# wangys16/FreeSplat

Measured on AMD Instinct MI355X. Metric: rendered views/sec @ 968x1296, 1.0M Gaussians, higher is better.
Workload: dtype f32

## Files before the change

freesplat_amd/csrc/raster_fwd.hip:

```cpp
#include <stdlib.h>

#include <type_traits>

#include "fs_common.h"
#include "raster_host.h"

namespace fs {

template <int M>
__device__ __forceinline__ uint32_t lane_xor(uint32_t v)
{
    if constexpr (M == 1) return (uint32_t)__builtin_amdgcn_mov_dpp((int)v, 0xB1, 0xF, 0xF, true);
    else if constexpr (M == 2) return (uint32_t)__builtin_amdgcn_mov_dpp((int)v, 0x4E, 0xF, 0xF, true);
    else if constexpr (M == 3) return (uint32_t)__builtin_amdgcn_mov_dpp((int)v, 0x1B, 0xF, 0xF, true);
    else if constexpr (M < 32) return (uint32_t)__builtin_amdgcn_ds_swizzle((int)v, (M << 10) | 0x1F);
    else return (uint32_t)__shfl_xor((int)v, M, 64);
}
template <int M>
__device__ __forceinline__ unsigned long long lane_xor64(unsigned long long v)
{
    const uint32_t lo = lane_xor<M>((uint32_t)v), hi = lane_xor<M>((uint32_t)(v >> 32));
    return ((unsigned long long)hi << 32) | lo;
}

// ... 200 lines not shown
        const float fx = (float)d.W / (2.0f * tanfovx), fy = (float)d.H / (2.0f * tanfovy);
        float c3[6];
#pragma unroll
        for (int k = 0; k < 6; ++k) c3[k] = c_in[k];
        if (rescale) {
            const float s2 = wscale * wscale;
#pragma unroll
            for (int k = 0; k < 6; ++k) c3[k] = c3[k] * s2;
        }
        const Cov2D cv = project_cov(view, p, c3, fx, fy, tanfovx, tanfovy);
        const float det = cv.a * cv.c - cv.b * cv.b;
        if (det != 0.0f) {
            const float det_inv = 1.0f / det;
            const float cA = cv.c * det_inv, cB = -cv.b * det_inv, cC = cv.a * det_inv;
            const float mid = 0.5f * (cv.a + cv.c);
            const float sq = sqrtf(fmaxf(0.1f, mid * mid - det));
            const float l1 = mid + sq, l2 = mid - sq;
            const float my_radius = ceilf(3.0f * sqrtf(fmaxf(l1, l2)));
            const float px = ((ndcx + 1.0f) * (float)d.W - 1.0f) * 0.5f;
            const float py = ((ndcy + 1.0f) * (float)d.H - 1.0f) * 0.5f;
            const int r = (int)my_radius;
            const int gx = (d.W + kTile - 1) / kTile, gy = (d.H + kTile - 1) / kTile;
            const int x0 = min(gx, max(0, (int)((px - (float)r) / (float)kTile)));
            const int y0 = min(gy, max(0, (int)((py - (float)r) / (float)kTile)));
            const int x1 = min(gx, max(0, (int)((px + (float)r + (float)(kTile - 1)) / (float)kTile)));
            const int y1 = min(gy, max(0, (int)((py + (float)r + (float)(kTile - 1)) / (float)kTile)));
            if ((x1 - x0) * (y1 - y0) > 0) {
                float rgb[3];
                if (colors) {
                    rgb[0] = colors[3 * i];
                    rgb[1] = colors[3 * i + 1];
                    rgb[2] = colors[3 * i + 2];
                } else {
                    float3 dir = make_float3(p.x - campos[0], p.y - campos[1], p.z - campos[2]);
                    const float len = sqrtf(dir.x * dir.x + dir.y * dir.y + dir.z * dir.z);
                    dir.x = dir.x / len; dir.y = dir.y / len; dir.z = dir.z / len;
                    switch (d.sh_degree) {
                        case 0: eval_sh<0>(sh, dir, rgb, o.cb, sh_cs, sh_ks); break;
                        case 1: eval_sh<1>(sh, dir, rgb, o.cb, sh_cs, sh_ks); break;
                        case 2: eval_sh<2>(sh, dir, rgb, o.cb, sh_cs, sh_ks); break;
                        default: eval_sh<3>(sh, dir, rgb, o.cb, sh_cs, sh_ks); break;
                    }
                }
                float thr;
                if (op > 0.0f) {
                    const float l = -logf(255.0f * op);
                    thr = l - (0.001f + 1e-5f * fabsf(l));
                } else {
                    thr = 1.0f;
                }
                o.r0 = make_float4(px, py, -0.5f * cA, -0.5f * cC);
                o.r1 = make_float4(-cB, op, thr, pv.z);
                o.r2 = make_float4(rgb[0], rgb[1], rgb[2], 0.0f);
                o.rect = make_ushort4((unsigned short)x0, (unsigned short)y0, (unsigned short)x1,
                                      (unsigned short)y1);
                o.rad = r;
            }
        }
    }
    return o;
}

template <bool SR>
__device__ __forceinline__ void load_mean_cov(const fs_raster_dims& d, const float* __restrict__ means3D,
                                              const float* __restrict__ cov3D, size_t i, float3& p_in, float (&c_in)[6])
{
    p_in = make_float3(means3D[3 * i], means3D[3 * i + 1], means3D[3 * i + 2]);
    if constexpr (SR) {
        float row[7];
#pragma unroll
        for (int k = 0; k < 7; ++k) row[k] = cov3D[7 * i + k];
        cov_from_scale_rot(row, c_in);
    } else if (d.flags & FS_RASTER_COV_FULL) {
        const float* cr = cov3D + 9 * i;
        c_in[0] = cr[0]; c_in[1] = cr[1]; c_in[2] = cr[2]; c_in[3] = cr[4]; c_in[4] = cr[5]; c_in[5] = cr[8];
    } else {
#pragma unroll
        for (int k = 0; k < 6; ++k) c_in[k] = cov3D[6 * i + k];
    }
}

constexpr int kWaveBins = 512;

__device__ __forceinline__ void bin_wave(const fs_raster_dims& d, int lane, uint32_t* s_cnt, uint32_t i, const Projected& pr,
                                         uint32_t* __restrict__ tile_counts, unsigned long long* __restrict__ keys,
                                         uint32_t tile_cap)
{
    const float4 r0 = pr.r0, r1 = pr.r1;
    const ushort4 rect = pr.rect;
    const bool valid = pr.rad > 0;
    const bool cull = (d.flags & FS_RASTER_TILE_CULL) != 0;
    const int gx = (d.W + kTile - 1) / kTile;
    const QuadForm qf = quad_form(r0, r1);
    const int rw = rect.z - rect.x, rh = rect.w - rect.y;
    const int area = rw * rh;
    const bool small = area <= 16;
    const bool all4 = __builtin_amdgcn_ballot_w64(valid && (rw > 4 || rh > 4)) == 0ull;
    unsigned long long qm = 0;
    uint32_t nz = 0u;
    if (all4) { if (valid) qm = pack_quad_masks4(qf, r0, rect, cull, nz); }
    else if (valid && small) qm = pack_quad_masks(qf, r0, rect);
    const unsigned long long key_hi = ((unsigned long long)__float_as_uint(r1.w) << 32) | (i << 4);
    int x0 = valid ? (int)rect.x : 0x7fff, y0 = valid ? (int)rect.y : 0x7fff;
    int x1 = valid ? (int)rect.z : 0, y1 = valid ? (int)rect.w : 0;
#define FS_BOX_STEP(M)                                                                                           \
    {                                                                                                            \
        const int lo = (int)lane_xor<M>((uint32_t)((x0 << 16) | y0)), hi = (int)lane_xor<M>((uint32_t)((x1 << 16) | y1)); \
        x0 = min(x0, lo >> 16); y0 = min(y0, lo & 0xffff);                                                       \
        x1 = max(x1, hi >> 16); y1 = max(y1, hi & 0xffff);                                                       \
    }
    FS_BOX_STEP(32) FS_BOX_STEP(16) FS_BOX_STEP(8) FS_BOX_STEP(4) FS_BOX_STEP(2) FS_BOX_STEP(1)
#undef FS_BOX_STEP
    const int bx0 = __builtin_amdgcn_readfirstlane(x0), by0 = __builtin_amdgcn_readfirstlane(y0);
    const int bw = max(0, __builtin_amdgcn_readfirstlane(x1) - bx0), bh = max(0, __builtin_amdgcn_readfirstlane(y1) - by0);
    const int nb = bw * bh;
    if (nb == 0) return;
    if (nb <= kWaveBins && all4) {
        for (int k = lane; k < nb; k += 64) s_cnt[k] = 0u;
        wave_lds_sync();
        const int cbase = (rect.y - by0) * bw + (rect.x - bx0);
        for (uint32_t z = nz; z != 0u; z &= z - 1u) {
            const int k = __builtin_ctz(z);
            atomicAdd(&s_cnt[cbase + (k >> 2) * bw + (k & 3)], 1u);
        }
        wave_lds_sync();
        for (int k0 = 0; k0 < nb; k0 += 64) {
            const int k = k0 + lane;
            if (k < nb) {
                const uint32_t c = s_cnt[k];
                const int ky = k / bw, kx = k - ky * bw;
                s_cnt[k] = c ? atomicAdd(&tile_counts[(by0 + ky) * gx + bx0 + kx], c) : 0u;
            }
        }
        wave_lds_sync();
        const uint32_t tbase = (uint32_t)(rect.y * gx + rect.x);
        for (uint32_t z = nz; z != 0u; z &= z - 1u) {
            const int k = __builtin_ctz(z);
            const uint32_t m = (uint32_t)(qm >> (4 * k)) & 15u;
            const uint32_t slot = atomicAdd(&s_cnt[cbase + (k >> 2) * bw + (k & 3)], 1u);
            if (slot < tile_cap) keys[(tbase + (uint32_t)((k >> 2) * gx + (k & 3))) * tile_cap + slot] = key_hi | m;
        }
        wave_lds_sync();
    } else if (nb <= kWaveBins) {
        for (int k = lane; k < nb; k += 64) s_cnt[k] = 0u;
        wave_lds_sync();
        if (valid) {
            int k = 0;
            for (int y = rect.y; y < rect.w; ++y) {
                RowBands rb = {};
                if (!small) rb = row_bands(qf, r0, y);
                for (int x = rect.x; x < rect.z; ++x, ++k) {
                    const uint32_t m = small ? (uint32_t)(qm >> (4 * k)) & 15u : quad_mask_row(rb, r0, x);
                    if (!cull || m) atomicAdd(&s_cnt[(y - by0) * bw + (x - bx0)], 1u);
                }
            }
        }
        wave_lds_sync();
        for (int k0 = 0; k0 < nb; k0 += 64) {
            const int k = k0 + lane;
            if (k < nb) {
                const uint32_t c = s_cnt[k];
                const int ky = k / bw, kx = k - ky * bw;
                s_cnt[k] = c ? atomicAdd(&tile_counts[(by0 + ky) * gx + bx0 + kx], c) : 0u;
            }
        }
        wave_lds_sync();
        if (valid) {
            int k = 0;
            for (int y = rect.y; y < rect.w; ++y) {
                RowBands rb = {};
                if (!small) rb = row_bands(qf, r0, y);
                for (int x = rect.x; x < rect.z; ++x, ++k) {
                    const uint32_t m = small ? (uint32_t)(qm >> (4 * k)) & 15u : quad_mask_row(rb, r0, x);
                    if (!cull || m) {
                        const uint32_t slot = atomicAdd(&s_cnt[(y - by0) * bw + (x - bx0)], 1u);
                        if (slot < tile_cap) keys[(uint32_t)(y * gx + x) * tile_cap + slot] = key_hi | m;
                    }
                }
            }
        }
        wave_lds_sync();
    } else if (all4) {
        const uint32_t tbase = (uint32_t)(rect.y * gx + rect.x);
        for (uint32_t z = nz; z != 0u; z &= z - 1u) {
            const int k = __builtin_ctz(z);
            const uint32_t m = (uint32_t)(qm >> (4 * k)) & 15u;
            const uint32_t tile = tbase + (uint32_t)((k >> 2) * gx + (k & 3));
            const uint32_t slot = atomicAdd(&tile_counts[tile], 1u);
            if (slot < tile_cap) keys[tile * tile_cap + slot] = key_hi | m;
        }
    } else if (valid) {
        int k = 0;
        for (int y = rect.y; y < rect.w; ++y) {
            RowBands rb = {};
            if (!small) rb = row_bands(qf, r0, y);
            for (int x = rect.x; x < rect.z; ++x, ++k) {
                const uint32_t m = small ? (uint32_t)(qm >> (4 * k)) & 15u : quad_mask_row(rb, r0, x);
                if (!cull || m) {
                    const uint32_t slot = atomicAdd(&tile_counts[y * gx + x], 1u);
                    if (slot < tile_cap) keys[(uint32_t)(y * gx + x) * tile_cap + slot] = key_hi | m;
                }
            }
        }
    }
}

__global__ __launch_bounds__(256) void zero_counts_kernel(char* base, size_t stride, int T)
{
    const int k = blockIdx.x * 256 + threadIdx.x;
    if (k < T) ((uint32_t*)(base + stride * blockIdx.y))[k] = 0u;
}

struct ViewBuffers {
    char* geom; size_t geom_stride;
    char* scratch; size_t scratch_stride;
    int32_t* radii;
};

#ifndef FS_PRE_WAVES
#define FS_PRE_WAVES 6
#endif
#define FS_PRE_OCC __attribute__((amdgpu_waves_per_eu(FS_PRE_WAVES, FS_PRE_WAVES)))
template <int CH, bool SR>
__global__ __launch_bounds__(256) FS_PRE_OCC void preprocess_views_kernel(
    fs_raster_dims d, int v, const float* __restrict__ means3D, const float* __restrict__ cov3D,
    const float* __restrict__ shs, const float* __restrict__ colors, const float* __restrict__ opacities,
    const float* __restrict__ view, const float* __restrict__ proj, const float* __restrict__ campos,
    const float* __restrict__ tanfov_dev, const float* __restrict__ scale_dev, ViewBuffers vb, uint32_t tile_cap)
{
    extern __shared__ __attribute__((aligned(16))) float lds[];
    constexpr int kPerBlock = 64 * CH;
    const int base = blockIdx.x * kPerBlock;
    const int cnt = min(kPerBlock, d.N - base);
    const int per_sh = shs ? d.M * 3 : 0;
    const bool sh_cm = (d.flags & FS_RASTER_SH_CHANNEL_MAJOR) != 0;
    const int sh_cs = sh_cm ? d.M : 1, sh_ks = sh_cm ? 1 : 3;
    float* const l_sh = lds;
    if (shs) {
        if (d.flags & FS_RASTER_SH_FP16) stage_rows_half(l_sh, (const _Float16*)shs, base, cnt, per_sh);
        else stage_rows(l_sh, shs, base, cnt, per_sh);
    }
    const int t = threadIdx.x, lane = t & 63, wave = t >> 6;
    const int chunk = wave % CH;
    uint32_t* const s_cnt_base = (uint32_t*)(lds + (size_t)kPerBlock * per_sh);
    uint32_t* const s_cnt = s_cnt_base + wave * kWaveBins;
    const int li = chunk * 64 + lane;
    const bool live = li < cnt;
    const uint32_t i = (uint32_t)(base + li);
    float* const l_g = (float*)(s_cnt_base + 4 * kWaveBins) + li;
    {
        float3 p_in = make_float3(0.0f, 0.0f, 0.0f);
        float c_in[6] = {0, 0, 0, 0, 0, 0};
        float op = 0.0f;
        if (live) {
            load_mean_cov<SR>(d, means3D, cov3D, i, p_in, c_in);
            op = opacities[i];
        }
        if (wave < CH) {
            l_g[0 * kPerBlock] = p_in.x; l_g[1 * kPerBlock] = p_in.y; l_g[2 * kPerBlock] = p_in.z;
#pragma unroll
            for (int k = 0; k < 6; ++k) l_g[(3 + k) * kPerBlock] = c_in[k];
            l_g[9 * kPerBlock] = op;
        }
    }
    __syncthreads();
    const int T = num_tiles(d.H, d.W);
    const size_t keys_off = align_up((size_t)T * 4, 256);
#pragma nounroll
    for (int j0 = wave / CH; j0 < v; j0 += 4 / CH) {
        const int j = __builtin_amdgcn_readfirstlane(j0);
        int li_ = li, lane_ = lane;
        asm volatile("" : "+v"(li_), "+v"(lane_));
        const float* const lg = (const float*)(s_cnt_base + 4 * kWaveBins) + li_;
        const float3 p_in = make_float3(lg[0 * kPerBlock], lg[1 * kPerBlock], lg[2 * kPerBlock]);
        float c_in[6];
#pragma unroll
        for (int k = 0; k < 6; ++k) c_in[k] = lg[(3 + k) * kPerBlock];
        const float op = lg[9 * kPerBlock];
        const float tanfovx = tanfov_dev ? tanfov_dev[2 * j] : d.tanfovx;
        const float tanfovy = tanfov_dev ? tanfov_dev[2 * j + 1] : d.tanfovy;
        const float wscale = scale_dev ? scale_dev[j] : 1.0f;
        const Projected pr = project_gaussian(d, live, p_in, c_in, op, i, colors, l_sh + (size_t)li_ * per_sh, sh_cs, sh_ks,
                                              view + 16 * j, proj + 16 * j, campos + 3 * j, tanfovx, tanfovy,
                                              scale_dev != nullptr, wscale);
        if (live) {
            const GeomView g = geom_view(vb.geom + vb.geom_stride * j, d.N);
            g.rec[3 * (size_t)i + 0] = pr.r0;
            g.rec[3 * (size_t)i + 1] = pr.r1;
            g.rec[3 * (size_t)i + 2] = pr.r2;
            if (!(d.flags & FS_RASTER_NO_BACKWARD_STATE)) {
                g.rect[i] = pr.rect;
                g.clamp[i] = pr.cb;
            }
            if (vb.radii) vb.radii[(size_t)j * d.N + i] = pr.rad;
        }
        char* const sc = vb.scratch + vb.scratch_stride * j;
        bin_wave(d, lane_, s_cnt, i, pr, (uint32_t*)sc, (unsigned long long*)(sc + keys_off), tile_cap);
    }
}

__global__ __launch_bounds__(1024) void tile_scan_kernel(const char* __restrict__ counts0, size_t counts_stride,
                                                         char* __restrict__ offsets0, size_t offsets_stride, int T,
                                                         uint32_t* __restrict__ counters0,
                                                         unsigned long long cap, uint32_t tile_cap)
{
    const uint32_t* __restrict__ counts = (const uint32_t*)(counts0 + counts_stride * blockIdx.x);
    uint32_t* __restrict__ offsets = (uint32_t*)(offsets0 + offsets_stride * blockIdx.x);
    uint32_t* __restrict__ counters = counters0 + 2 * blockIdx.x;
    __shared__ uint32_t s_wave[16];
    __shared__ uint32_t s_max[16];
    __shared__ unsigned long long s_wide[16];
    const int t = threadIdx.x, lane = t & 63, wave = t >> 6;
    const int per = (T + 1023) / 1024;
    const int lo = min(T, t * per), hi = min(T, lo + per);
    uint32_t s = 0, mx = 0;
    unsigned long long wide = 0;
    for (int k = lo; k < hi; ++k) { const uint32_t c = counts[k]; s += c; wide += c; mx = max(mx, c); }
#pragma unroll
    for (int d = 32; d >= 1; d >>= 1) {
        wide += __shfl_xor(wide, d, 64);
        mx = max(mx, (uint32_t)__shfl_xor((int)mx, d, 64));
    }
    if (lane == 0) { s_wide[wave] = wide; s_max[wave] = mx; }
    uint32_t inc = s;
#pragma unroll
    for (int d = 1; d < 64; d <<= 1) {
        const uint32_t o = __shfl_up(inc, d, 64);
        if (lane >= d) inc += o;
    }
    if (lane == 63) s_wave[wave] = inc;
    __syncthreads();
    uint32_t before = 0, total = 0;
#pragma unroll
    for (int k = 0; k < 16; ++k) {
        const uint32_t v = s_wave[k];
        before += k < wave ? v : 0u;
        total += v;
    }
    inc += before;
    uint32_t run = inc - s;
    for (int k = lo; k < hi; ++k) {
        offsets[k] = run;
        run += counts[k];
    }
    if (t == 1023) {
        unsigned long long total64 = 0;
        uint32_t maxc = 0;
#pragma unroll
        for (int k = 0; k < 16; ++k) { total64 += s_wide[k]; maxc = max(maxc, s_max[k]); }
        offsets[T] = total;
        counters[0] = total64 > 0xFFFFFFFFull ? 0xFFFFFFFFu : (uint32_t)total64;
        counters[1] = (total64 > cap || maxc > tile_cap) ? max(maxc, 1u) : 0u;
    }
}

#ifndef FS_SORT_LDS
#define FS_SORT_LDS 1792
#endif
constexpr int kSortLds = FS_SORT_LDS;

template <typename Ptr>
__device__ __forceinline__ void bitonic_sort_any(Ptr a, uint32_t n)
{
    uint32_t P = 1;
    while (P < n) P <<= 1;
    const uint32_t half = P >> 1;
    for (uint32_t k = 2; k <= P; k <<= 1) {
        const uint32_t hk = k >> 1;
        for (uint32_t t = threadIdx.x; t < half; t += blockDim.x) {
            const uint32_t blk = t / hk, off = t % hk;
            const uint32_t i = blk * k + off, j = blk * k + (k - 1 - off);
            if (j < n) {
                const unsigned long long x = a[i], y = a[j];
                if (x > y) { a[i] = y; a[j] = x; }
            }
        }
        __syncthreads();
        for (uint32_t s = k >> 2; s >= 1; s >>= 1) {
            for (uint32_t t = threadIdx.x; t < half; t += blockDim.x) {
                const uint32_t i = (t / s) * 2 * s + (t % s), j = i + s;
                if (j < n) {
                    const unsigned long long x = a[i], y = a[j];
                    if (x > y) { a[i] = y; a[j] = x; }
                }
            }
            __syncthreads();
        }
    }
}

template <int EPT, int TM, bool REV>
__device__ __forceinline__ void thread_exchange(unsigned long long (&k)[EPT], int t, unsigned long long* lds)
{
    constexpr int HB = TM >= 128 ? 128 : TM >= 64 ? 64 : TM >= 32 ? 32 : TM >= 16 ? 16 : TM >= 8 ? 8 : TM >= 4 ? 4 : TM >= 2 ? 2 : 1;
    const bool low = (t & HB) == 0;
    unsigned long long y[EPT];
    if constexpr (TM < 64) {
#pragma unroll
        for (int e = 0; e < EPT; ++e) y[e] = lane_xor64<TM>(k[REV ? EPT - 1 - e : e]);
    } else {
        constexpr int CH = EPT * 256 > kSortLds ? kSortLds / 256 : EPT;
#pragma unroll
        for (int e0 = 0; e0 < EPT; e0 += CH) {
            __syncthreads();
#pragma unroll
            for (int e = 0; e < CH; ++e) lds[e * 256 + t] = k[REV ? EPT - 1 - (e0 + e) : e0 + e];
            __syncthreads();
#pragma unroll
            for (int e = 0; e < CH; ++e) y[e0 + e] = lds[e * 256 + (t ^ TM)];
        }
    }
#pragma unroll
    for (int e = 0; e < EPT; ++e) {
        const unsigned long long x = k[e];
        k[e] = low ? (y[e] < x ? y[e] : x) : (y[e] > x ? y[e] : x);
    }
}

template <int EPT, int J>
struct Clean {
    static __device__ __forceinline__ void run(unsigned long long (&k)[EPT], int t, unsigned long long* lds)
    {
        if constexpr (J >= EPT) {
            thread_exchange<EPT, J / EPT, false>(k, t, lds);
        } else {
#pragma unroll
            for (int e = 0; e < EPT; ++e)
                if ((e & J) == 0) {
                    const unsigned long long a = k[e], b = k[e | J];
                    if (a > b) { k[e] = b; k[e | J] = a; }
                }
        }
        if constexpr (J > 1) Clean<EPT, J / 2>::run(k, t, lds);
    }
};
template <int EPT, int K>
struct Stages {
    static __device__ __forceinline__ void run(unsigned long long (&k)[EPT], int t, unsigned long long* lds)
    {
        if constexpr (K > 2) Stages<EPT, K / 2>::run(k, t, lds);
        if constexpr (K <= EPT) {
#pragma unroll
            for (int e = 0; e < EPT; ++e) {
                const int p = e ^ (K - 1);
                if (e < p) {
                    const unsigned long long a = k[e], b = k[p];
                    if (a > b) { k[e] = b; k[p] = a; }
                }
            }
        } else {
            thread_exchange<EPT, K / EPT - 1, true>(k, t, lds);
        }
        if constexpr (K >= 4) Clean<EPT, K / 4>::run(k, t, lds);
    }
};

constexpr uint32_t kMaxBucket = 24;
template <int EPT>
__device__ __forceinline__ void sort_tile_buckets(const unsigned long long* keys, uint32_t* __restrict__ gout,
                                                  uint32_t n, unsigned long long* sk, uint32_t* cnt, uint32_t* s_red,
                                                  int tid = -1)
{
    constexpr int CAP = 256 * EPT;
    uint32_t* const list = cnt;
    const int t = tid >= 0 ? tid : (int)threadIdx.x, lane = t & 63, wave = t >> 6;
    unsigned long long k[EPT];
    uint32_t zmin = 0xFFFFFFFFu, zmax = 0u;
#pragma unroll
    for (int e = 0; e < EPT; ++e) {
        const uint32_t i = (uint32_t)(e * 256 + t);
        k[e] = i < n ? keys[i] : ~0ull;
        cnt[i] = 0u;
        if (i < n) {
            const uint32_t z = (uint32_t)(k[e] >> 32);
            zmin = min(zmin, z);
            zmax = max(zmax, z);
        }
    }
    if (t == 0) cnt[CAP] = 0u;
#pragma unroll
    for (int m = 32; m >= 1; m >>= 1) {
        zmin = min(zmin, (uint32_t)__shfl_xor((int)zmin, m, 64));
        zmax = max(zmax, (uint32_t)__shfl_xor((int)zmax, m, 64));
    }
    if (lane == 0) { s_red[wave] = zmin; s_red[4 + wave] = zmax; }
    __syncthreads();
    zmin = min(min(s_red[0], s_red[1]), min(s_red[2], s_red[3]));
    zmax = max(max(s_red[4], s_red[5]), max(s_red[6], s_red[7]));
    const float scale = (float)CAP / (float)(zmax - zmin + 1u);
    uint32_t bs[EPT];
#pragma unroll
    for (int e = 0; e < EPT; ++e) {
        const uint32_t i = (uint32_t)(e * 256 + t);
        bs[e] = 0u;
        if (i < n) {
            const uint32_t z = (uint32_t)(k[e] >> 32);
            const uint32_t b = min((uint32_t)(CAP - 1), (uint32_t)((float)(z - zmin) * scale));
            const uint32_t slot = atomicAdd(&cnt[b], 1u);
            bs[e] = (b << 8) | min(slot, 255u);
        }
    }
    __syncthreads();
    uint32_t c[EPT], sum = 0u, mx = 0u;
#pragma unroll
    for (int j = 0; j < EPT; ++j) {
        c[j] = cnt[t * EPT + j];
        sum += c[j];
        mx = max(mx, c[j]);
    }
    uint32_t inc = sum;
#pragma unroll
    for (int d = 1; d < 64; d <<= 1) {
        const uint32_t o = (uint32_t)__shfl_up((int)inc, d, 64);
        if (lane >= d) inc += o;
    }
    if (lane == 63) s_red[8 + wave] = inc;
    const bool degenerate = __syncthreads_or(mx > kMaxBucket) != 0;
    uint32_t run = inc - sum;
#pragma unroll
    for (int w = 0; w < 3; ++w) run += w < wave ? s_red[8 + w] : 0u;
    if (degenerate) {
        if constexpr ((EPT & (EPT - 1)) == 0) {
            Stages<EPT, CAP>::run(k, t, sk);
            __syncthreads();
#pragma unroll
            for (int e = 0; e < EPT; ++e) {
                const uint32_t i = (uint32_t)t * EPT + e;
                if (i < n) {
                    list[i] = (uint32_t)k[e];
                    if (gout) gout[i] = (uint32_t)k[e];
                }
            }
        } else {
            __syncthreads();
#pragma unroll
            for (int e = 0; e < EPT; ++e)
                if ((uint32_t)(e * 256 + t) < n) sk[e * 256 + t] = k[e];
            __syncthreads();
            bitonic_sort_any(sk, n);
            for (uint32_t i = (uint32_t)t; i < n; i += 256u) {
                const uint32_t wd = (uint32_t)sk[i];
                list[i] = wd;
                if (gout) gout[i] = wd;
            }
        }
        return;
    }
#pragma unroll
    for (int j = 0; j < EPT; ++j) {
        cnt[t * EPT + j] = run;
        run += c[j];
    }
    if (t == 255) cnt[CAP] = run;
    __syncthreads();
#pragma unroll
    for (int e = 0; e < EPT; ++e)
        if ((uint32_t)(e * 256 + t) < n) sk[cnt[bs[e] >> 8] + (bs[e] & 255u)] = k[e];
    __syncthreads();
    uint32_t pos[EPT];
#pragma unroll
    for (int e = 0; e < EPT; ++e) {
        pos[e] = 0u;
        if ((uint32_t)(e * 256 + t) < n) {
            const uint32_t b = bs[e] >> 8;
            const uint32_t lo = cnt[b], hi = cnt[b + 1];
            uint32_t r = 0u;
            for (uint32_t j = lo; j < hi; ++j) r += sk[j] < k[e] ? 1u : 0u;
            pos[e] = lo + r;
        }
    }
    __syncthreads();
#pragma unroll
    for (int e = 0; e < EPT; ++e) {
        if ((uint32_t)(e * 256 + t) < n) {
            list[pos[e]] = (uint32_t)k[e];
            if (gout) gout[pos[e]] = (uint32_t)k[e];
        }
    }
}

constexpr int kMaxGroups = 64;
__device__ __forceinline__ bool sort_tile_partitioned(
    const unsigned long long* __restrict__ kt, uint32_t* __restrict__ gl, uint32_t n,
                                                      unsigned long long* sk, uint32_t* cnt, uint32_t* s_red, uint32_t* s_grp)
{
    constexpr int NB = kSortLds;
    const int t = threadIdx.x, lane = t & 63, wave = t >> 6;
    uint32_t zmin = 0xFFFFFFFFu, zmax = 0u;
    for (uint32_t i = t; i < n; i += 256) {
        const uint32_t z = (uint32_t)(kt[i] >> 32);
        zmin = min(zmin, z);
        zmax = max(zmax, z);
    }
    for (int i = t; i <= NB; i += 256) cnt[i] = 0u;
#pragma unroll
    for (int m = 32; m >= 1; m >>= 1) {
        zmin = min(zmin, (uint32_t)__shfl_xor((int)zmin, m, 64));
        zmax = max(zmax, (uint32_t)__shfl_xor((int)zmax, m, 64));
    }
    if (lane == 0) { s_red[wave] = zmin; s_red[4 + wave] = zmax; }
    __syncthreads();
    zmin = min(min(s_red[0], s_red[1]), min(s_red[2], s_red[3]));
    zmax = max(max(s_red[4], s_red[5]), max(s_red[6], s_red[7]));
// ... 180 lines not shown
    auto next_batch = [&]() __attribute__((always_inline)) -> int {
        while (c < n) {
            const bool hit = (w_cur & qbit) != 0;
            const unsigned long long hits = __ballot(hit);
            const uint32_t w_hit = w_cur;
            const uint32_t e = (uint32_t)(c + lane);
            w_cur = w_nxt;
            w_nxt = c + 128 + lane < n ? pl[c + 128 + lane] : 0u;
            c += 64;
            if (!hits) continue;
            const int slot = filled + __builtin_amdgcn_mbcnt_hi((uint32_t)(hits >> 32), __builtin_amdgcn_mbcnt_lo((uint32_t)hits, 0));
            if (hit && slot < 64) {
                qi[slot] = e;
                if constexpr (!LDS_LIST) qw[slot] = w_hit;
            }
            filled += __popcll(hits);
            if (filled >= 64) {
                take(64);
                if (hit && slot >= 64) {
                    qi[slot - 64] = e;
                    if constexpr (!LDS_LIST) qw[slot - 64] = w_hit;
                }
                filled -= 64;
                return 64;
            }
        }
        const int cnt = filled;
        if (cnt != 0) take(cnt);
        filled = 0;
        return cnt;
    };
    int rem = 0, cur = 0;
    for (;;) {
        if (done_m == ~0ull) break;
        if (lane < cur) {
            const int k = rem + lane;
            float* d = (float*)(cp + (k >> 1) * kPairQuads) + (k & 1);
            d[0] = r0.x; d[2] = r0.y;
            d[4] = -r0.z; d[6] = -r0.w;
            d[8] = -r1.x; d[10] = skip_bits(r1.z);
            d[12] = r1.y;
            if constexpr (TRACK) d[14] = __int_as_float(r_pos);
            cp[(k >> 1) * kPairQuads + 4 + (k & 1)] = make_float4(r2.x, r2.y, r2.z, r1.w);
        }
        const int nxt = next_batch();
        if (cur != 0) {
            wave_lds_sync();
            const int total = rem + cur, nfull = total >> 2;
            for (int p = 0; p < nfull; ++p) {
                if (done_m == ~0ull) break;
                step(cp + 2 * p * kPairQuads, std::false_type{}, 4);
            }
            rem = total & 3;
            if (rem != 0 && nfull != 0) {
                float4 t = {};
                if (lane < 2 * kPairQuads) t = cp[2 * nfull * kPairQuads + lane];
                if (lane < 2 * kPairQuads) cp[lane] = t;
            }
            wave_lds_sync();
        }
        cur = nxt;
        if (cur == 0) break;
    }
    if (rem != 0 && done_m != ~0ull) {
        if (lane >= rem && lane < 4) cp[(lane >> 1) * kPairQuads + 4 + (lane & 1)] = make_float4(0.0f, 0.0f, 0.0f, 0.0f);
        wave_lds_sync();
        step(cp, std::true_type{}, rem);
    }
#undef FS_BLEND_ONE
    if (inside) {
        const int ln = __builtin_amdgcn_mbcnt_hi(~0u, __builtin_amdgcn_mbcnt_lo(~0u, 0));
        const int ox = tx * kTile + (wave & 1) * 8 + (ln & 7), oy = ty * kTile + (wave >> 1) * 8 + (ln >> 3);
        const size_t pix = (size_t)oy * W + ox, HW = (size_t)H * W;
        final_T[pix] = T_;
        if constexpr (TRACK) n_contrib[pix] = last;
        out_color[pix] = fmaf(T_, bg[0], C01.x);
        out_color[HW + pix] = fmaf(T_, bg[1], C01.y);
        out_color[2 * HW + pix] = fmaf(T_, bg[2], C2D.x);
        out_depth[pix] = C2D.y;
        out_alpha[pix] = 1.0f - T_;
    }
}

static_assert(4 * (kPairArea * sizeof(float4) + 64 * sizeof(uint32_t)) <= kSortLds * sizeof(unsigned long long),
              "compaction areas and hit queues must fit the key staging");
template <bool FAST_EXP, bool TRACK>
#ifndef FS_BLEND_WAVES
#define FS_BLEND_WAVES 7
#endif
__global__ __launch_bounds__(256) __attribute__((amdgpu_waves_per_eu(FS_BLEND_WAVES, FS_BLEND_WAVES))) void sort_blend_kernel(
    int H, int W, const uint32_t* __restrict__ counts, const uint32_t* __restrict__ offsets, uint32_t tile_cap,
    unsigned long long* __restrict__ keys, uint32_t* __restrict__ point_list, const float4* __restrict__ rec,
    const float* __restrict__ bg, const uint32_t* __restrict__ counters,
    float* __restrict__ out_color, float* __restrict__ out_depth, float* __restrict__ out_alpha,
    float* __restrict__ final_T, int32_t* __restrict__ n_contrib)
{
    __shared__ __attribute__((aligned(16))) unsigned long long sk[kSortLds];
    __shared__ uint32_t s_cnt[kSortLds + 1];
    __shared__ uint32_t s_red[16];
    __shared__ uint32_t s_grp[2 * kMaxGroups + 3];
    if (counters[1]) return;
    const int gx = (W + kTile - 1) / kTile, gy = (H + kTile - 1) / kTile;
    const int tile = tile_for_block(blockIdx.x, gx, gy);
    if (tile < 0) return;
    FS_PT(2, 0);
    const uint32_t n = counts[tile];
    unsigned long long* const kt = keys + (size_t)tile * tile_cap;
    uint32_t* const gl = point_list + offsets[tile];
    const bool in_lds = n <= (uint32_t)kSortLds;
    if (n == 0) {
    } else if (n <= 256u) {
        sort_tile_buckets<1>(kt, TRACK ? gl : nullptr, n, sk, s_cnt, s_red);
    } else if (n <= 512u) {
        sort_tile_buckets<2>(kt, TRACK ? gl : nullptr, n, sk, s_cnt, s_red);
    } else if (n <= 1024u) {
        sort_tile_buckets<4>(kt, TRACK ? gl : nullptr, n, sk, s_cnt, s_red);
    } else if (n <= (uint32_t)kSortLds) {
        sort_tile_buckets<kSortLds / 256>(kt, TRACK ? gl : nullptr, n, sk, s_cnt, s_red);
    }
    else if (!sort_tile_partitioned(kt, gl, n, sk, s_cnt, s_red, s_grp)) {
        __syncthreads();
        bitonic_sort_any(kt, n);
        for (uint32_t k = threadIdx.x; k < n; k += 256) gl[k] = (uint32_t)kt[k];
    }
    if (!in_lds) __threadfence_block();
    FS_PT(2, 1);
    __syncthreads();
    FS_PT(2, 2);
    const int wave = __builtin_amdgcn_readfirstlane(threadIdx.x >> 6);
    float4* const cp = (float4*)sk + wave * kPairArea;
    uint32_t* const qi = (uint32_t*)((float4*)sk + 4 * kPairArea) + wave * 64;
    uint32_t* const qw = s_cnt + wave * 64;
    const int tx = tile % gx, ty = tile / gx;
    if (in_lds)
        blend_quadrant<FAST_EXP, TRACK, true>(s_cnt, (int)n, rec, cp, qi, nullptr, H, W, tx, ty, wave, bg, out_color, out_depth, out_alpha,
                                              final_T, n_contrib);
    else
        blend_quadrant<FAST_EXP, TRACK, false>(gl, (int)n, rec, cp, qi, qw, H, W, tx, ty, wave, bg, out_color, out_depth, out_alpha,
                                               final_T, n_contrib);
    FS_PT(2, 3);
}

}

using namespace fs;

FS_API int fs_raster_buffer_sizes(int32_t N, int32_t H, int32_t W, int64_t cap, size_t out[4])
{
    if (N < 0 || H <= 0 || W <= 0 || cap < 0 || !out) return FS_ERR_INVALID_ARG;
    out[0] = geom_bytes(N > 0 ? N : 1);
    out[1] = BinningLayout(H, W, cap).total;
    out[2] = ImageLayout(H, W).total;
    out[3] = FwdScratchLayout(H, W, cap).total;
    return FS_OK;
}

FS_API const uint32_t* fs_raster_tile_ranges(const void* binning, int32_t, int32_t)
{
    return (const uint32_t*)binning;
}
FS_API const uint32_t* fs_raster_point_list(const void* binning, int32_t H, int32_t W)
{
    return at<const uint32_t>(binning, BinningLayout(H, W).point_list);
}
FS_API const float* fs_raster_geom_records(const void* geom) { return (const float*)geom; }
FS_API const float* fs_raster_final_T(const void* image) { return (const float*)image; }
FS_API const int32_t* fs_raster_n_contrib(const void* image, int32_t H, int32_t W)
{
    return at<const int32_t>(image, ImageLayout(H, W).n_contrib);
}

namespace fs {
static int raster_batch()
{
    static const int n = [] {
        const char* e = getenv("FREESPLAT_RASTER_BATCH");
        const int x = e ? atoi(e) : 16;
        return x < 1 ? 1 : (x > kMaxViewsInFlight ? kMaxViewsInFlight : x);
    }();
    return n;
}

static int check_forward_args(bool required, const fs_raster_dims& d, const float* means3D, const float* cov3D, const float* shs,
                              const float* colors_precomp, const float* opacities, const int32_t* radii, int64_t cap)
{
    if (!required) return FS_ERR_INVALID_ARG;
    if (d.N < 0 || d.H <= 0 || d.W <= 0 || cap < 1) return FS_ERR_INVALID_ARG;
    if ((d.flags & FS_RASTER_SCALE_ROT) && (d.flags & FS_RASTER_COV_FULL)) return FS_ERR_INVALID_ARG;
    if (d.N > 0) {
        if (!means3D || !cov3D || !opacities || !radii) return FS_ERR_INVALID_ARG;
        if ((shs == nullptr) == (colors_precomp == nullptr)) return FS_ERR_INVALID_ARG;
    }
    if (shs && (d.sh_degree < 0 || d.sh_degree > 3 || (d.sh_degree + 1) * (d.sh_degree + 1) > d.M))
        return FS_ERR_UNSUPPORTED;
    const int gx = (d.W + kTile - 1) / kTile, gy = (d.H + kTile - 1) / kTile;
    if (gx > 32767 || gy > 32767) return FS_ERR_UNSUPPORTED;
    if (d.N > (1 << 28)) return FS_ERR_UNSUPPORTED;
    if (cap > 0xFFFFFFFFll) return FS_ERR_UNSUPPORTED;
    return FS_OK;
}

static int launch_binning(const fs_raster_dims& d, int nv, const float* means3D, const float* cov3D, const float* shs,
                          const float* colors_precomp, const float* opacities, const float* viewmatrix,
                          const float* projmatrix, const float* campos, const float* tanfov, const float* scale,
                          void* geom, size_t geom_stride, void* binning, size_t binning_stride, void* scratch,
                          size_t scratch_stride, int64_t cap, int32_t* radii, uint32_t* counters, hipStream_t st)
{
    const FwdScratchLayout sl(d.H, d.W, cap);
    const int T = sl.T;
    const uint32_t tile_cap = sl.tile_cap;
    hipLaunchKernelGGL(zero_counts_kernel, dim3((T + 255) / 256, nv), dim3(256), 0, st, (char*)scratch, scratch_stride, T);
    FS_CHECK_LAUNCH("zero tile counts");
    if (d.N > 0) {
        const int M = shs ? d.M : 0;
// ... 172 lines not shown
```

profiles/phase_trace.py:

```python
#!/usr/bin/env python
import ctypes as C
import os
import sys

import numpy as np
import torch

ROOT = os.path.dirname(os.path.dirname(os.path.abspath(__file__)))
sys.path.insert(0, ROOT)
from freesplat_amd import _lib, synthetic
from freesplat_amd.decoder import render_views

PHASES = {
    0: ("preprocess (projection + binning)", ["stage inputs + sync", "project / conic / SH", "write records + sync", "quadrant masks",
                       "workgroup box", "zero + count (LDS atomics)", "reserve slots (returning global atomics)",
                       "rank + write keys"]),
    2: ("sort_blend (wavefront 0)", ["load keys + LDS bucket sort", "wait for the other wavefronts", "blend quadrant 0"]),
}


def main():
    dev = torch.device("cuda:0")
    H, W, N = synthetic.WORKLOADS["c3_968x1296_1M"]
    scene = synthetic.make_scene(N)
    cams = {k: v[:1].to(dev) for k, v in synthetic.target_cameras(8).items()}
    g = {k: scene[k].to(dev) for k in ("means", "covariances", "harmonics", "opacities")}
    L = _lib.lib()
    L.fs_debug_phase_trace.restype = C.c_int
    buf = np.zeros(4 * 4096 * 10, np.uint64)
    with torch.no_grad():
        for it in range(4):
            render_views(cams["extrinsics"], cams["intrinsics"], cams["near"], cams["far"], (H, W), torch.zeros(1, 3, device=dev),
                         g["means"], g["covariances"], g["harmonics"], g["opacities"])
            torch.cuda.synchronize()
            L.fs_debug_phase_trace(buf.ctypes.data_as(C.c_void_p))
    t = buf.reshape(4, 4096, 10).astype(np.float64) / 100.0
    for kern, (name, phases) in PHASES.items():
        n = len(phases) + 1
        x = t[kern][:, :n]
        x = x[(x > 0).all(axis=1)]
        if not len(x):
            print(f"{name}: no samples")
            continue
        d = np.diff(x, axis=1)
        print(f"{name}: {len(x)} workgroups, {(x[:, -1] - x[:, 0]).mean():.2f} us each")
        for ph, m, md in zip(phases, d.mean(0), np.median(d, 0)):
            print(f"   {ph:34s} mean {m:6.2f} us   median {md:6.2f}")


if __name__ == "__main__":
    main()
```

Before: 4680.

## Pack sort/blend LDS into one arena and shrink sort staging for occupancy

Replaces the four separate shared arrays of the sort+blend kernel with a single byte arena whose regions are laid out explicitly, and lowers the LDS key-staging capacity so the total fits eight workgroups per CU. The bucket-sort degeneracy check now folds a wave ballot into the high bit of the per-wave prefix total, using a plain barrier instead of __syncthreads_or. The aim is higher occupancy and a cheaper barrier. In exchange, more tiles exceed the smaller LDS capacity and take the slower global-memory partitioned sort path.

```diff
diff --git a/freesplat_amd/csrc/raster_fwd.hip b/freesplat_amd/csrc/raster_fwd.hip
--- a/freesplat_amd/csrc/raster_fwd.hip
+++ b/freesplat_amd/csrc/raster_fwd.hip
@@ -579,9 +579,10 @@
 }
 
 #ifndef FS_SORT_LDS
-#define FS_SORT_LDS 1792
+#define FS_SORT_LDS 1536
 #endif
 constexpr int kSortLds = FS_SORT_LDS;
+static_assert(kSortLds % 256 == 0 && kSortLds > 1024, "the LDS sort's capacity is a multiple of the workgroup's 256 threads");
 
 template <typename Ptr>
 __device__ __forceinline__ void bitonic_sort_any(Ptr a, uint32_t n)
@@ -738,11 +739,14 @@
         const uint32_t o = (uint32_t)__shfl_up((int)inc, d, 64);
         if (lane >= d) inc += o;
     }
-    if (lane == 63) s_red[8 + wave] = inc;
-    const bool degenerate = __syncthreads_or(mx > kMaxBucket) != 0;
+    const uint32_t wdeg = __builtin_amdgcn_ballot_w64(mx > kMaxBucket) != 0ull ? 0x80000000u : 0u;
+    if (lane == 63) s_red[8 + wave] = inc | wdeg;
+    __syncthreads();
+    const uint32_t tot[4] = {s_red[8], s_red[9], s_red[10], s_red[11]};
+    const bool degenerate = (((tot[0] | tot[1]) | (tot[2] | tot[3])) >> 31) != 0u;
     uint32_t run = inc - sum;
 #pragma unroll
-    for (int w = 0; w < 3; ++w) run += w < wave ? s_red[8 + w] : 0u;
+    for (int w = 0; w < 3; ++w) run += w < wave ? tot[w] & 0x7FFFFFFFu : 0u;
     if (degenerate) {
         if constexpr ((EPT & (EPT - 1)) == 0) {
             Stages<EPT, CAP>::run(k, t, sk);
@@ -1089,8 +1093,24 @@
     }
 }
 
-static_assert(4 * (kPairArea * sizeof(float4) + 64 * sizeof(uint32_t)) <= kSortLds * sizeof(unsigned long long),
-              "compaction areas and hit queues must fit the key staging");
+constexpr size_t kGrpWords = 2 * kMaxGroups + 3;
+constexpr size_t kArenaList = 0;
+constexpr size_t kArenaStage = ((kSortLds + 1) * sizeof(uint32_t) + 15) / 16 * 16;
+constexpr size_t kArenaStageEnd = kArenaStage + kSortLds * sizeof(unsigned long long);
+constexpr size_t kArenaQueues = kArenaStage + 4 * kPairArea * sizeof(float4);
+constexpr size_t kArenaBlendEnd = kArenaQueues + 4 * 64 * sizeof(uint32_t);
+constexpr size_t kArenaRed = kArenaStageEnd;
+constexpr size_t kArenaGrp = kArenaRed + 16 * sizeof(uint32_t);
+constexpr size_t kArenaSortEnd = kArenaGrp + kGrpWords * sizeof(uint32_t);
+constexpr size_t kArenaBytes = (kArenaBlendEnd > kArenaSortEnd ? kArenaBlendEnd : kArenaSortEnd);
+static_assert(kArenaList + (kSortLds + 1) * sizeof(uint32_t) <= kArenaStage, "list / bucket offsets end before the staging");
+static_assert(kArenaStage % 16 == 0, "the staging holds 64-bit keys and the float4 compaction areas");
+static_assert(kArenaQueues % 16 == 0 && kArenaRed % 4 == 0 && kArenaGrp % 4 == 0, "alignment of the overlaid arrays");
+static_assert(kArenaRed >= kArenaStageEnd, "the sort's small arrays must not overlap its key staging");
+static_assert(4 * 64 * sizeof(uint32_t) <= (kSortLds + 1) * sizeof(uint32_t), "the global-list path's hit words fit the list's words");
+#if FS_SORT_LDS <= 1536
+static_assert(kArenaBytes <= 20480, "eight workgroups per CU (160 KiB of LDS)");
+#endif
 template <bool FAST_EXP, bool TRACK>
 #ifndef FS_BLEND_WAVES
 #define FS_BLEND_WAVES 7
@@ -1102,10 +1122,11 @@
     float* __restrict__ out_color, float* __restrict__ out_depth, float* __restrict__ out_alpha,
     float* __restrict__ final_T, int32_t* __restrict__ n_contrib)
 {
-    __shared__ __attribute__((aligned(16))) unsigned long long sk[kSortLds];
-    __shared__ uint32_t s_cnt[kSortLds + 1];
-    __shared__ uint32_t s_red[16];
-    __shared__ uint32_t s_grp[2 * kMaxGroups + 3];
+    __shared__ __attribute__((aligned(16))) unsigned char arena[kArenaBytes];
+    uint32_t* const s_cnt = (uint32_t*)(arena + kArenaList);
+    unsigned long long* const sk = (unsigned long long*)(arena + kArenaStage);
+    uint32_t* const s_red = (uint32_t*)(arena + kArenaRed);
+    uint32_t* const s_grp = (uint32_t*)(arena + kArenaGrp);
     if (counters[1]) return;
     const int gx = (W + kTile - 1) / kTile, gy = (H + kTile - 1) / kTile;
     const int tile = tile_for_block(blockIdx.x, gx, gy);
@@ -1136,7 +1157,7 @@
     FS_PT(2, 2);
     const int wave = __builtin_amdgcn_readfirstlane(threadIdx.x >> 6);
     float4* const cp = (float4*)sk + wave * kPairArea;
-    uint32_t* const qi = (uint32_t*)((float4*)sk + 4 * kPairArea) + wave * 64;
+    uint32_t* const qi = (uint32_t*)(arena + kArenaQueues) + wave * 64;
     uint32_t* const qw = s_cnt + wave * 64;
     const int tx = tile % gx, ty = tile / gx;
     if (in_lds)
```

New measurement: 4708 (median of 6 runs). Within noise of the previous version (+0.6%).

## Defer record stores behind reserve atomics and rank keys per quad row

Applied to the files above, without the earlier changes.

Restructures the all-4x4 binning path in bin_wave. LDS counting now happens per quad row with returned ranks packed into registers, so the key-writing pass can drop its second round of LDS atomics. The global geometry-record stores are moved into a callback issued after the first returning tile_counts atomic, so their latency overlaps the reservation. Partial chunks are excluded from the fast path, and the slot index uses a shift and a float reciprocal instead of a multiply and integer divide. Phase-trace probes and profiler script updates are added. The code assumes tile_cap is a power of two, and the float-reciprocal division could misround for some bw values.

```diff
diff --git a/freesplat_amd/csrc/raster_fwd.hip b/freesplat_amd/csrc/raster_fwd.hip
--- a/freesplat_amd/csrc/raster_fwd.hip
+++ b/freesplat_amd/csrc/raster_fwd.hip
@@ -306,9 +306,11 @@
 
 constexpr int kWaveBins = 512;
 
+template <bool B> struct BoolTag { static constexpr bool value = B; };
+template <class StoreRecord>
 __device__ __forceinline__ void bin_wave(const fs_raster_dims& d, int lane, uint32_t* s_cnt, uint32_t i, const Projected& pr,
                                          uint32_t* __restrict__ tile_counts, unsigned long long* __restrict__ keys,
-                                         uint32_t tile_cap)
+                                         uint32_t tile_cap, bool full_chunk, const StoreRecord& store_record)
 {
     const float4 r0 = pr.r0, r1 = pr.r1;
     const ushort4 rect = pr.rect;
@@ -319,7 +321,7 @@
     const int rw = rect.z - rect.x, rh = rect.w - rect.y;
     const int area = rw * rh;
     const bool small = area <= 16;
-    const bool all4 = __builtin_amdgcn_ballot_w64(valid && (rw > 4 || rh > 4)) == 0ull;
+    const bool all4 = full_chunk && __builtin_amdgcn_ballot_w64(valid && (rw > 4 || rh > 4)) == 0ull;
     unsigned long long qm = 0;
     uint32_t nz = 0u;
     if (all4) { if (valid) qm = pack_quad_masks4(qf, r0, rect, cull, nz); }
@@ -338,32 +340,69 @@
     const int bx0 = __builtin_amdgcn_readfirstlane(x0), by0 = __builtin_amdgcn_readfirstlane(y0);
     const int bw = max(0, __builtin_amdgcn_readfirstlane(x1) - bx0), bh = max(0, __builtin_amdgcn_readfirstlane(y1) - by0);
     const int nb = bw * bh;
+    const bool ranked = nb != 0 && nb <= kWaveBins && all4;
+    if (!ranked) store_record(BoolTag<false>());
     if (nb == 0) return;
-    if (nb <= kWaveBins && all4) {
+    if (ranked) {
         for (int k = lane; k < nb; k += 64) s_cnt[k] = 0u;
         wave_lds_sync();
         const int cbase = (rect.y - by0) * bw + (rect.x - bx0);
-        for (uint32_t z = nz; z != 0u; z &= z - 1u) {
-            const int k = __builtin_ctz(z);
-            atomicAdd(&s_cnt[cbase + (k >> 2) * bw + (k & 3)], 1u);
-        }
+        uint32_t zv = 0u;
+        asm volatile("" : "+v"(zv));
+        uint32_t rk[4];
+#pragma unroll
+        for (int r = 0; r < 4; ++r) {
+            const uint32_t row = (nz >> (4 * r)) & 15u;
+            rk[r] = 0u;
+            if (__builtin_amdgcn_ballot_w64(row != 0u) == 0ull) continue;
+            uint32_t* const c_row = s_cnt + (cbase + __mul24(r, bw));
+            uint32_t q[4] = {zv, zv, zv, zv};
+#pragma unroll
+            for (int c = 0; c < 4; ++c)
+                if (row & (1u << c)) q[c] = atomicAdd(&c_row[c], 1u);
+            rk[r] = q[0] | (q[1] << 8) | (q[2] << 16) | (q[3] << 24);
+        }
+        FS_PT(0, 3);
         wave_lds_sync();
-        for (int k0 = 0; k0 < nb; k0 += 64) {
+        const float rbw = __builtin_amdgcn_rcpf((float)bw);
+        const auto counter_tile = [&](int k) {
+            const int ky = (int)(((float)k + 0.5f) * rbw);
+            return (by0 + ky) * gx + bx0 + (k - __mul24(ky, bw));
+        };
+        for (int k0 = 64; k0 < nb; k0 += 64) {
             const int k = k0 + lane;
-            if (k < nb) {
-                const uint32_t c = s_cnt[k];
-                const int ky = k / bw, kx = k - ky * bw;
-                s_cnt[k] = c ? atomicAdd(&tile_counts[(by0 + ky) * gx + bx0 + kx], c) : 0u;
-            }
-        }
+            const uint32_t c = k < nb ? s_cnt[k] : 0u;
+            if (c) s_cnt[k] = atomicAdd(&tile_counts[counter_tile(k)], c);
+        }
+        {
+            const uint32_t c = lane < nb ? s_cnt[lane] : 0u;
+            uint32_t first = 0u;
+            if (c) first = atomicAdd(&tile_counts[counter_tile(lane)], c);
+            store_record(BoolTag<true>());
+            if (c) s_cnt[lane] = first;
+        }
+        FS_PT(0, 4);
         wave_lds_sync();
         const uint32_t tbase = (uint32_t)(rect.y * gx + rect.x);
-        for (uint32_t z = nz; z != 0u; z &= z - 1u) {
-            const int k = __builtin_ctz(z);
-            const uint32_t m = (uint32_t)(qm >> (4 * k)) & 15u;
-            const uint32_t slot = atomicAdd(&s_cnt[cbase + (k >> 2) * bw + (k & 3)], 1u);
-            if (slot < tile_cap) keys[(tbase + (uint32_t)((k >> 2) * gx + (k & 3))) * tile_cap + slot] = key_hi | m;
-        }
+        const int cap_shift = 31 - __builtin_clz(tile_cap);
+#pragma unroll
+        for (int r = 0; r < 4; ++r) {
+            const uint32_t row = (nz >> (4 * r)) & 15u;
+            if (__builtin_amdgcn_ballot_w64(row != 0u) == 0ull) continue;
+            const uint32_t* const c_row = s_cnt + (row ? cbase + __mul24(r, bw) : 0);
+            uint32_t first[4];
+#pragma unroll
+            for (int c = 0; c < 4; ++c) first[c] = c_row[c];
+            const uint32_t t_row = tbase + (uint32_t)__mul24(r, gx);
+            const uint32_t m_row = (uint32_t)(qm >> (16 * r));
+#pragma unroll
+            for (int c = 0; c < 4; ++c) {
+                const uint32_t slot = first[c] + ((rk[r] >> (8 * c)) & 255u);
+                if ((row & (1u << c)) && slot < tile_cap)
+                    keys[((t_row + (uint32_t)c) << cap_shift) + slot] = key_hi | ((m_row >> (4 * c)) & 15u);
+            }
+        }
+        FS_PT(0, 5);
         wave_lds_sync();
     } else if (nb <= kWaveBins) {
         for (int k = lane; k < nb; k += 64) s_cnt[k] = 0u;
@@ -493,6 +532,7 @@
 #pragma nounroll
     for (int j0 = wave / CH; j0 < v; j0 += 4 / CH) {
         const int j = __builtin_amdgcn_readfirstlane(j0);
+        FS_PT(0, 0);
         int li_ = li, lane_ = lane;
         asm volatile("" : "+v"(li_), "+v"(lane_));
         const float* const lg = (const float*)(s_cnt_base + 4 * kWaveBins) + li_;
@@ -507,19 +547,27 @@
         const Projected pr = project_gaussian(d, live, p_in, c_in, op, i, colors, l_sh + (size_t)li_ * per_sh, sh_cs, sh_ks,
                                               view + 16 * j, proj + 16 * j, campos + 3 * j, tanfovx, tanfovy,
                                               scale_dev != nullptr, wscale);
+        FS_PT(0, 1);
         if (live) {
-            const GeomView g = geom_view(vb.geom + vb.geom_stride * j, d.N);
-            g.rec[3 * (size_t)i + 0] = pr.r0;
-            g.rec[3 * (size_t)i + 1] = pr.r1;
-            g.rec[3 * (size_t)i + 2] = pr.r2;
             if (!(d.flags & FS_RASTER_NO_BACKWARD_STATE)) {
+                const GeomView g = geom_view(vb.geom + vb.geom_stride * j, d.N);
                 g.rect[i] = pr.rect;
                 g.clamp[i] = pr.cb;
             }
             if (vb.radii) vb.radii[(size_t)j * d.N + i] = pr.rad;
         }
+        const auto store_record = [&](auto full) {
+            if (decltype(full)::value || live) {
+                const GeomView g = geom_view(vb.geom + vb.geom_stride * j, d.N);
+                g.rec[3 * (size_t)i + 0] = pr.r0;
+                g.rec[3 * (size_t)i + 1] = pr.r1;
+                g.rec[3 * (size_t)i + 2] = pr.r2;
+            }
+            FS_PT(0, 2);
+        };
         char* const sc = vb.scratch + vb.scratch_stride * j;
-        bin_wave(d, lane_, s_cnt, i, pr, (uint32_t*)sc, (unsigned long long*)(sc + keys_off), tile_cap);
+        bin_wave(d, lane_, s_cnt, i, pr, (uint32_t*)sc, (unsigned long long*)(sc + keys_off), tile_cap,
+                 (chunk + 1) * 64 <= cnt, store_record);
     }
 }
 
diff --git a/profiles/phase_trace.py b/profiles/phase_trace.py
--- a/profiles/phase_trace.py
+++ b/profiles/phase_trace.py
@@ -12,9 +12,8 @@
 from freesplat_amd.decoder import render_views
 
 PHASES = {
-    0: ("preprocess (projection + binning)", ["stage inputs + sync", "project / conic / SH", "write records + sync", "quadrant masks",
-                       "workgroup box", "zero + count (LDS atomics)", "reserve slots (returning global atomics)",
-                       "rank + write keys"]),
+    0: ("preprocess_views (wavefront 0, last view)", ["projection", "record stores issued", "count walk done (masks, box, zero, count)",
+                                                      "reserve atomics returned", "key walk done"]),
     2: ("sort_blend (wavefront 0)", ["load keys + LDS bucket sort", "wait for the other wavefronts", "blend quadrant 0"]),
 }
 
@@ -23,14 +22,15 @@
     dev = torch.device("cuda:0")
     H, W, N = synthetic.WORKLOADS["c3_968x1296_1M"]
     scene = synthetic.make_scene(N)
-    cams = {k: v[:1].to(dev) for k, v in synthetic.target_cameras(8).items()}
+    views = int(sys.argv[1]) if len(sys.argv) > 1 else 16
+    cams = {k: v[:views].to(dev) for k, v in synthetic.target_cameras(max(views, 8)).items()}
     g = {k: scene[k].to(dev) for k in ("means", "covariances", "harmonics", "opacities")}
     L = _lib.lib()
     L.fs_debug_phase_trace.restype = C.c_int
     buf = np.zeros(4 * 4096 * 10, np.uint64)
     with torch.no_grad():
         for it in range(4):
-            render_views(cams["extrinsics"], cams["intrinsics"], cams["near"], cams["far"], (H, W), torch.zeros(1, 3, device=dev),
+            render_views(cams["extrinsics"], cams["intrinsics"], cams["near"], cams["far"], (H, W), torch.zeros(views, 3, device=dev),
                          g["means"], g["covariances"], g["harmonics"], g["opacities"])
             torch.cuda.synchronize()
             L.fs_debug_phase_trace(buf.ctypes.data_as(C.c_void_p))
@@ -42,10 +42,13 @@
         if not len(x):
             print(f"{name}: no samples")
             continue
+        order = [0] + [int(k) + 1 for k in np.argsort(np.median(x[:, 1:] - x[:, :1], axis=0), kind="stable")]
+        x = x[:, order]
+        x = x[(np.diff(x, axis=1) >= 0).all(axis=1)]
         d = np.diff(x, axis=1)
         print(f"{name}: {len(x)} workgroups, {(x[:, -1] - x[:, 0]).mean():.2f} us each")
-        for ph, m, md in zip(phases, d.mean(0), np.median(d, 0)):
-            print(f"   {ph:34s} mean {m:6.2f} us   median {md:6.2f}")
+        for k, m, md in zip(order[1:], d.mean(0), np.median(d, 0)):
+            print(f"   -> {phases[k - 1]:44s} mean {m:6.2f} us   median {md:6.2f}")
 
 
 if __name__ == "__main__":
```

After: 4644 before, 4673 after (median of 6 runs). About the same (+0.6%).
